# microsoft/vattention

Hardware: AMD Instinct MI355X
Metric: prefill+decode tokens/sec (attention + KV-memory hot path) (higher is better)
Workload: dtype f16

## Files before the change

vattention_amd/csrc/prefill64_common.h:

```cpp
#pragma once
#include "attn_common.h"

namespace vattn_k {

typedef float f32x2 __attribute__((ext_vector_type(2)));
constexpr float kDeferLog2 = 6.0f;

__device__ __forceinline__ void dma_piece(unsigned lds_addr, u32x4 rsrc, unsigned voff) {
    asm volatile("s_mov_b32 m0, %0\n\ts_nop 0\n\tbuffer_load_dwordx4 %2, %1, 0 offen lds" : : "s"(lds_addr), "s"(rsrc), "v"(voff) : "memory", "m0");
}
__device__ __forceinline__ void dma_piece_first(unsigned lds_addr, u32x4 rsrc, unsigned voff) {
    asm volatile("s_nop 4\n\ts_mov_b32 m0, %0\n\ts_nop 0\n\tbuffer_load_dwordx4 %2, %1, 0 offen lds" : : "s"(lds_addr), "s"(rsrc), "v"(voff) : "memory", "m0");
}
template <int OFF> __device__ __forceinline__ void dma_piece_at(unsigned lds_base, u32x4 rsrc, unsigned voff) {
    asm volatile("s_add_u32 m0, %0, %3\n\ts_nop 0\n\tbuffer_load_dwordx4 %2, %1, 0 offen lds" : : "s"(lds_base), "s"(rsrc), "v"(voff), "i"(OFF) : "memory", "m0", "scc");
}
template <int OFF, int ROWS> __device__ __forceinline__ void dma_piece_so(unsigned lds_base, u32x4 rsrc, unsigned voff, unsigned row_bytes) {
    unsigned so;
    asm volatile("s_add_u32 m0, %1, %6\n\ts_mul_i32 %0, %4, %5\n\tbuffer_load_dwordx4 %3, %2, %0 offen lds"
                 : "=&s"(so) : "s"(lds_base), "s"(rsrc), "v"(voff), "s"(row_bytes), "n"(ROWS), "i"(OFF) : "memory", "m0", "scc");
}
template <int ROWS> __device__ __forceinline__ unsigned piece_off(unsigned base, unsigned row_bytes) {
    unsigned r;
    asm("v_mad_u32_u24 %0, %1, %3, %2" : "=v"(r) : "s"(row_bytes), "v"(base), "n"(ROWS));
    return r;
}
__device__ __forceinline__ void k_rsrc_advance(u32x4& r, int& rows_left, unsigned tile_bytes, unsigned row_bytes) {
    asm volatile("s_add_u32 s92, s92, %3\n\ts_addc_u32 s93, s93, 0\n\ts_sub_i32 %1, %1, 64\n\ts_min_i32 s94, %1, 64\n\ts_max_i32 s94, s94, 0\n\ts_mul_i32 s94, s94, %4"
                 : "={s[92:95]}"(r), "+s"(rows_left) : "0"(r), "s"(tile_bytes), "s"(row_bytes) : "scc");
}
__device__ __forceinline__ void v_rsrc_advance(u32x4& r, int& rows_left, unsigned tile_bytes, unsigned row_bytes) {
    asm volatile("s_add_u32 s96, s96, %3\n\ts_addc_u32 s97, s97, 0\n\ts_sub_i32 %1, %1, 64\n\ts_min_i32 s98, %1, 64\n\ts_max_i32 s98, s98, 0\n\ts_mul_i32 s98, s98, %4"
                 : "={s[96:99]}"(r), "+s"(rows_left) : "0"(r), "s"(tile_bytes), "s"(row_bytes) : "scc");
}
__device__ __forceinline__ u32x4 tile_rsrc(const void* base, unsigned bytes) {
    const unsigned long long a = (unsigned long long)base;
    u32x4 r;
    r[0] = __builtin_amdgcn_readfirstlane((unsigned)a);
    r[1] = __builtin_amdgcn_readfirstlane((unsigned)(a >> 32)) & 0xffffu;
    r[2] = __builtin_amdgcn_readfirstlane(bytes);
    r[3] = 0x00020000u;
    return r;
}

template <typename T> struct Mfma;
#define VATTN_MFMA_STRUCT(TYPE, MNEM)                                                                                                    \
    template <> struct Mfma<TYPE> {                                                                                                \
        using V8 = typename Tr<TYPE>::v8;                                                                                          \
                                                                   \
        static __device__ __forceinline__ void qk_first(f32x16& d, V8 a, V8 b) {                                                   \
            asm volatile(MNEM " %0, %1, %2, 0" : "=&v"(d) : "v"(a), "a"(b));                                                       \
        }                                                                                                                          \
        static __device__ __forceinline__ void qk_acc(f32x16& d, V8 a, V8 b) {                                                     \
            asm volatile(MNEM " %0, %1, %2, %0" : "+v"(d) : "v"(a), "a"(b));                                                       \
        }                                                                                                                          \
                                                           \
        static __device__ __forceinline__ void qk_first_a(f32x16& d, V8 a, V8 b) {                                                 \
            asm volatile(MNEM " %0, %1, %2, 0" : "=&v"(d) : "a"(a), "a"(b));                                                       \
        }                                                                                                                          \
        static __device__ __forceinline__ void qk_acc_a(f32x16& d, V8 a, V8 b) {                                                   \
            asm volatile(MNEM " %0, %1, %2, %0" : "+v"(d) : "a"(a), "a"(b));                                                       \
        }                                                                                                                          \
                                                                                                 \
        static __device__ __forceinline__ void pv(f32x16& o, V8 a, V8 b) {                                                         \
            asm volatile(MNEM " %0, %1, %2, %0" : "+a"(o) : "v"(a), "v"(b));                                                       \
        }                                                                                                                          \
    };
VATTN_MFMA_STRUCT(_Float16, "v_mfma_f32_32x32x16_f16")
VATTN_MFMA_STRUCT(__bf16, "v_mfma_f32_32x32x16_bf16")
#undef VATTN_MFMA_STRUCT
__device__ __forceinline__ float add1(float a, float b) {
    float r;
    asm("v_add_f32 %0, %1, %2" : "=v"(r) : "v"(a), "v"(b));
    return r;
}
#define SCHED_FENCE() __builtin_amdgcn_sched_barrier(0)

constexpr int kKPiece = 1088;
constexpr int kKSlot = 16 * 1088;
constexpr int kVBase = 36864;

template <typename V8> __device__ __forceinline__ V8 kfrag(const char* ksm, int f, unsigned kfrag_lane) {
    const int kk = f >> 1, kb = f & 1;
    return *(const V8*)(ksm + kb * 8 * kKPiece + kk * 128 + kfrag_lane);
}
template <typename V8> __device__ __forceinline__ V8 vfrag(const char* vsm, int f, unsigned vfrag_lane) {
    const int ks = f >> 2, db = f & 3;
    const char* a1 = vsm + db * PfSmem<128>::kVSubBytes + (16 * ks) * 64 + vfrag_lane;
    const s16x4 lo = __builtin_amdgcn_ds_read_tr16_b64_v4i16(LDS_PTR(s16x4, a1));
    const s16x4 hi = __builtin_amdgcn_ds_read_tr16_b64_v4i16(LDS_PTR(s16x4, a1 + 8 * 64));
    return join_tr<V8>(lo, hi);
}
__device__ __forceinline__ float row_max(const f32x16 (&s)[2][2], int qc) {
    float m0 = fmaxf(s[0][qc][0], s[1][qc][0]);
#pragma unroll
    for (int r = 1; r < 16; r++) m0 = fmaxf(fmaxf(m0, s[0][qc][r]), s[1][qc][r]);
    return fmaxf(m0, swap_halves(m0));
}
template <int DB> __device__ __forceinline__ void raise_max(f32x16 (&o)[DB][2], float (&l_acc)[2][2], float (&nmsub)[2], int qc, float delta) {
    const float alpha = fast_exp2(-delta);
    nmsub[qc] -= delta;
#pragma unroll
    for (int i = 0; i < DB; i++)
#pragma unroll
        for (int r = 0; r < 16; r++) o[i][qc][r] *= alpha;
#pragma unroll
    for (int a4 = 0; a4 < 2; a4++) l_acc[qc][a4] *= alpha;
}
template <typename T> __device__ __forceinline__ typename Tr<T>::v8 pack_p(const f32x16 (&pt)[2][2], int ks, int qc) {
    typename Tr<T>::v8 r;
#pragma unroll
    for (int j = 0; j < 8; j++) r[j] = Tr<T>::cvt(pt[ks >> 1][qc][8 * (ks & 1) + j]);
    return r;
}
__device__ __forceinline__ unsigned bound(int rows, unsigned rs) {
    int r;
    asm("s_min_i32 %0, %1, 64\n\ts_max_i32 %0, %0, 0" : "=s"(r) : "s"(rows) : "scc");
    return (unsigned)r * rs;
}

template <int NA> __device__ __forceinline__ void softmax_stages(int G, f32x16 (&cur)[2][2], float (&l_acc)[2][2], const float (&nmsub)[2], unsigned escale_s) {
    auto GE = [](int e) { return e < NA ? 1 + (e * 30) / NA : 33 + ((e - NA) * 17) / (32 - NA); };
#define P64_X0(cur, e) cur[(e) >> 4][((e) >> 2) & 1][8 * (((e) >> 3) & 1) + 2 * ((e) & 3)]
#define P64_X1(cur, e) cur[(e) >> 4][((e) >> 2) & 1][8 * (((e) >> 3) & 1) + 2 * ((e) & 3) + 1]
#pragma unroll
    for (int e = 0; e < 32; e++) {
        const int qc = (e >> 2) & 1;
        if (GE(e) - 1 == G)
            asm("v_fma_f32 %0, %0, %2, %3\n\tv_fma_f32 %1, %1, %2, %3" : "+v"(P64_X0(cur, e)), "+v"(P64_X1(cur, e)) : "s"(escale_s), "v"(nmsub[qc]));
        if (GE(e) == G) asm("v_exp_f32 %0, %0\n\tv_exp_f32 %1, %1" : "+v"(P64_X0(cur, e)), "+v"(P64_X1(cur, e)));
        if (GE(e) + 1 == G)
            asm("v_add_f32 %0, %0, %2\n\tv_add_f32 %1, %1, %3" : "+v"(l_acc[qc][0]), "+v"(l_acc[qc][1]) : "v"(P64_X0(cur, e)), "v"(P64_X1(cur, e)));
    }
#undef P64_X0
#undef P64_X1
}

template <typename T, int KK> __device__ __forceinline__ void first_scores(const char* ksm, f32x16 (&sc)[2][2], const typename Tr<T>::v8 (&qf)[2][KK], unsigned kfrag_lane) {
    using V8 = typename Tr<T>::v8;
    using M = Mfma<T>;
#pragma unroll
    for (int f = 0; f < 2 * KK; f++) {
        const V8 a = kfrag<V8>(ksm, f, kfrag_lane);
#pragma unroll
        for (int qc = 0; qc < 2; qc++) {
            if (f < 2) M::qk_first(sc[f & 1][qc], a, qf[qc][f >> 1]);
            else M::qk_acc(sc[f & 1][qc], a, qf[qc][f >> 1]);
        }
    }
    asm volatile("s_nop 15\n\ts_nop 3" ::: "memory");
    SCHED_FENCE();
}

struct StepMax {
    float mx0, mx1, g0, g1, grow;
};
template <typename T, int NA, int RING, int MS, int BJ, int D0, int DS, typename Hook>
__device__ __forceinline__ StepMax tile_step(const int par, const char* smem, f32x16 (&cur)[2][2], f32x16 (&nxt)[2][2], typename Tr<T>::v8& kf0,
                                             typename Tr<T>::v8& kf1, typename Tr<T>::v8& kf2, const typename Tr<T>::v8 (&qf)[2][8], f32x16 (&o)[4][2],
                                             float (&l_acc)[2][2], const float (&nmsub)[2], u32x4& rk, u32x4& rv, int& k_rows_left, int& v_rows_left,
                                             unsigned& vs_cur, unsigned& vs_dma, unsigned k_lds_wave, unsigned v_lds_wave, unsigned koff, unsigned voff,
                                             unsigned k_rs_bytes, unsigned v_rs_bytes, unsigned k_tile_b, unsigned v_tile_b, unsigned kfrag_lane,
                                             unsigned vfrag_lane, unsigned escale_s, Hook hook) {
    using V8 = typename Tr<T>::v8;
    using M = Mfma<T>;
    using S = PfSmem<128>;
    constexpr int KK = 8;
    static_assert(D0 >= BJ && D0 + 7 * DS < 32, "DMA pieces behind the barrier, inside phase B");
    static_assert(NA >= 16 && NA < 32, "key slice 0 of P is packed in phase-A groups 13 / 15: its eight pairs must be exponentiated by group 12");
    static_assert(MS >= 4 && MS + 19 < 32, "row-max chain >= 4 MFMAs behind the last S^T MFMA, its reduction inside phase B");
    auto dma_gap = [](int k) { return D0 + DS * k; };
    const int s_cur = par;
    const char* ksm = smem + (s_cur ^ 1) * kKSlot;
    const char* ksm_next = smem + s_cur * kKSlot;
    const char* vsm = smem + kVBase + vs_cur;
    const unsigned lk0 = k_lds_wave + (unsigned)((s_cur ^ 1) * kKSlot);
    unsigned lv0 = 0;
    V8 pf[2][2];
    V8 kf[RING];
    V8 vf[RING];
    SCHED_FENCE();
#pragma unroll
    for (int i = 0; i < 32; i++) {
        const int f = i >> 1, qc = i & 1;
        if (f < RING - 1) {
            const V8 a = f == 0 ? kf0 : (f == 1 ? kf1 : kf2);
            if (i < 4) M::qk_first_a(nxt[f & 1][qc], a, qf[qc][f >> 1]);
            else M::qk_acc_a(nxt[f & 1][qc], a, qf[qc][f >> 1]);
        } else if (i < 4) M::qk_first(nxt[f & 1][qc], kf[f % RING], qf[qc][f >> 1]);
        else M::qk_acc(nxt[f & 1][qc], kf[f % RING], qf[qc][f >> 1]);
        if ((i & 1) == 0 && f + RING - 1 < 2 * KK) kf[(f + RING - 1) % RING] = kfrag<V8>(ksm, f + RING - 1, kfrag_lane);
        softmax_stages<NA>(i, cur, l_acc, nmsub, escale_s);
        if (i == 13) pf[0][0] = pack_p<T>(cur, 0, 0);
        if (i == 15) pf[0][1] = pack_p<T>(cur, 0, 1);
        if (i == 17) lv0 = v_lds_wave + vs_dma;
        if (i == 19) asm volatile("s_mov_b32 %1, %0\n\ts_add_u32 %0, %0, %2\n\ts_cmp_eq_u32 %0, %3\n\ts_cselect_b32 %0, 0, %0"
                                  : "+s"(vs_cur), "=&s"(vs_dma) : "i"(S::kTileBytes), "i"(3 * S::kTileBytes) : "scc");
        if (i == 21) k_rsrc_advance(rk, k_rows_left, k_tile_b, k_rs_bytes);
        if (i == 23) v_rsrc_advance(rv, v_rows_left, v_tile_b, v_rs_bytes);
        hook(i);
        if (i == 26) vf[0] = vfrag<V8>(vsm, 0, vfrag_lane);
        if (i == 28) vf[1] = vfrag<V8>(vsm, 1, vfrag_lane);
        if (i == 30 && RING > 3) vf[2] = vfrag<V8>(vsm, 2, vfrag_lane);
        SCHED_FENCE();
    }
    float mx0 = -INFINITY, mx1 = -INFINITY, g0 = -INFINITY, g1 = -INFINITY, grow = -INFINITY;
    SCHED_FENCE();
#pragma unroll
    for (int j = 0; j < 32; j++) {
        const int f = j >> 1, ks = j >> 3, qc = j & 1;
        if (j == BJ) {
            asm volatile("s_waitcnt vmcnt(0)" ::: "memory");
            __builtin_amdgcn_s_barrier();
        }
        M::pv(o[f & 3][qc], vf[f % RING], pf[ks & 1][qc]);
        if ((j & 1) == 0 && f + RING - 1 < 16) vf[(f + RING - 1) % RING] = vfrag<V8>(vsm, f + RING - 1, vfrag_lane);
        softmax_stages<NA>(32 + j, cur, l_acc, nmsub, escale_s);
        if (ks < 3 && (j & 7) == 4) pf[(ks + 1) & 1][0] = pack_p<T>(cur, ks + 1, 0);
        if (ks < 3 && (j & 7) == 6) pf[(ks + 1) & 1][1] = pack_p<T>(cur, ks + 1, 1);
        if (j >= MS && j < MS + 16) {
            const int r = j - MS;
            if (r == 0) {
                asm("v_max_f32_e32 %0, %1, %2" : "=v"(mx0) : "v"(nxt[0][0][0]), "v"(nxt[1][0][0]));
                asm("v_max_f32_e32 %0, %1, %2" : "=v"(mx1) : "v"(nxt[0][1][0]), "v"(nxt[1][1][0]));
            } else {
                asm("v_max3_f32 %0, %0, %1, %2" : "+v"(mx0) : "v"(nxt[0][0][r]), "v"(nxt[1][0][r]));
                asm("v_max3_f32 %0, %0, %1, %2" : "+v"(mx1) : "v"(nxt[0][1][r]), "v"(nxt[1][1][r]));
            }
        }
        if (j == MS + 16) mx0 = max_halves(mx0);
        if (j == MS + 17) mx1 = max_halves(mx1);
        if (j == MS + 18) {
            asm("v_fma_f32 %0, %2, %4, %5\n\tv_fma_f32 %1, %3, %4, %6" : "=&v"(g0), "=&v"(g1) : "v"(mx0), "v"(mx1), "s"(escale_s), "v"(nmsub[0]), "v"(nmsub[1]));
        }
        if (j == MS + 19) asm("v_max_f32 %0, %1, %2" : "=v"(grow) : "v"(g0), "v"(g1));
        if (j == dma_gap(0)) dma_piece_at<0>(lk0, rk, koff);
        if (j == dma_gap(1)) dma_piece_so<kKPiece, 4>(lk0, rk, koff, k_rs_bytes);
        if (j == dma_gap(2)) dma_piece_so<2 * kKPiece, 8>(lk0, rk, koff, k_rs_bytes);
        if (j == dma_gap(3)) dma_piece_so<3 * kKPiece, 12>(lk0, rk, koff, k_rs_bytes);
        if (j == dma_gap(4)) dma_piece_at<0>(lv0, rv, voff);
        if (j == dma_gap(5)) dma_piece_so<1024, 16>(lv0, rv, voff, v_rs_bytes);
        if (j == dma_gap(6)) dma_piece_so<2048, 32>(lv0, rv, voff, v_rs_bytes);
        if (j == dma_gap(7)) dma_piece_so<3072, 48>(lv0, rv, voff, v_rs_bytes);
        if (j == 27) kf0 = kfrag<V8>(ksm_next, 0, kfrag_lane);
        if (j == 28) kf1 = kfrag<V8>(ksm_next, 1, kfrag_lane);
        if (j == 29 && RING > 3) kf2 = kfrag<V8>(ksm_next, 2, kfrag_lane);
        SCHED_FENCE();
    }
    return {mx0, mx1, g0, g1, grow};
}

}
```

vattention_amd/csrc/prefill64_kernel.inc:

```
template <typename T>
__global__ __launch_bounds__(256, 1) void P64_KERNEL_NAME(vattn_attn_params p, int order, int nqb, int nsplit) {
    constexpr bool WIN = P64_WIN;
    constexpr int NA = 24, RING = 4, MS = 8, BJ = 8, D0 = 9, DS = 3;
    using X = Tr<T>;
    using V8 = typename X::v8;
    constexpr int HD = 128;
    using S = PfSmem<HD>;
    constexpr int BM = 256;
    constexpr int KK = HD / 16;
    constexpr int DB = HD / 32;
    extern __shared__ __attribute__((aligned(16))) char smem[];

    const int tid = threadIdx.x;
    const int lane = tid & 63;
    const int wave = __builtin_amdgcn_readfirstlane(tid >> 6);
    const int l31 = lane & 31;
    const int g = lane >> 5;

    int b, h, qb, split;
    const bool listed = p.pf_items != nullptr;
    int it_tb = 0, it_te = 0, it_row = -1;
    if (listed) {
        const vattn_prefill_item it = p.pf_items[blockIdx.x];
        b = __builtin_amdgcn_readfirstlane(it.b);
        h = __builtin_amdgcn_readfirstlane(it.h);
        qb = __builtin_amdgcn_readfirstlane(it.qb);
        it_tb = __builtin_amdgcn_readfirstlane(it.tile_begin);
        it_te = __builtin_amdgcn_readfirstlane(it.tile_end);
        it_row = __builtin_amdgcn_readfirstlane(it.nshares > 1 ? it.part_row : -1);
        split = 0;
    } else if (!wg_to_work(p, order, nqb, nsplit, b, h, qb, split)) return;
    const bool partial = listed ? it_row >= 0 : nsplit > 1;
    const int hk = h / (p.h / p.h_k);
    const int slot = __builtin_amdgcn_readfirstlane(p.cache_batch_idx ? p.cache_batch_idx[b] : b);
    int Lk = __builtin_amdgcn_readfirstlane((p.cache_seqlens ? p.cache_seqlens[b] : p.seqlen_k) + p.seqlen_knew);
    Lk = Lk > p.seqlen_k ? p.seqlen_k : Lk;
    const int Sq = p.q_lens ? __builtin_amdgcn_readfirstlane(p.q_lens[b]) : p.seqlen_q;
    const int64_t q_first = p.q_start ? (int64_t)__builtin_amdgcn_readfirstlane(p.q_start[b]) : 0;
    const bool causal = p.is_causal != 0;
    const int off = Lk - Sq;
    const int q_wg0 = qb * BM;
    if (q_wg0 >= Sq) return;
    const int qw0 = q_wg0 + wave * 64;

    int n_end = Lk;
    if (causal) n_end = min(Lk, q_wg0 + BM + off);
    if (n_end < 0) n_end = 0;
    const int nt_all = (n_end + PF_BN - 1) / PF_BN;
    const int left = WIN ? p.window_left_plus1 - 1 : 0;
    const int t_first = WIN ? min(nt_all, max(0, q_wg0 + off - left) >> 6) : 0;
    int tb = t_first, nt = nt_all;
    if (listed) {
        tb = min(nt_all, it_tb);
        nt = min(nt_all, it_te);
    } else if (nsplit > 1) {
        const int per = (nt_all - t_first + nsplit - 1) / nsplit;
        tb = min(nt_all, t_first + split * per);
        nt = min(nt_all, tb + per);
    }
    const T* kbase = uniform_ptr((const T*)p.k_cache + (int64_t)slot * p.k_batch_stride + (int64_t)hk * p.k_head_stride);
    const T* vbase = uniform_ptr((const T*)p.v_cache + (int64_t)slot * p.v_batch_stride + (int64_t)hk * p.v_head_stride);
    const unsigned k_rs_bytes = (unsigned)p.k_row_stride * 2u, v_rs_bytes = (unsigned)p.v_row_stride * 2u;

    unsigned koff[4], voff[4];
#pragma unroll
    for (int j = 0; j < 4; j++) {
        const int row = 4 * (4 * wave + j) + (lane & 3);
        koff[j] = (unsigned)row * k_rs_bytes + (unsigned)((lane >> 2) << 4);
        const int key = 16 * j + (lane >> 2);
        voff[j] = (unsigned)key * v_rs_bytes + (unsigned)((4 * wave + (lane & 3)) << 4);
    }
    const unsigned k_lds_wave = (unsigned)(wave * 4 * kKPiece);
    const unsigned v_lds_wave = (unsigned)(kVBase + wave * 4096);
    auto kslot = [&](int t) { return (t - tb) & 1; };
    auto k_rsrc = [&](int t) -> u32x4 {
        int rem = Lk - t * PF_BN;
        rem = rem < 0 ? 0 : (rem > PF_BN ? PF_BN : rem);
        return tile_rsrc(kbase + (int64_t)t * PF_BN * p.k_row_stride, (unsigned)rem * k_rs_bytes);
    };
    auto v_rsrc = [&](int t) -> u32x4 {
        int rem = Lk - t * PF_BN;
        rem = rem < 0 ? 0 : (rem > PF_BN ? PF_BN : rem);
        return tile_rsrc(vbase + (int64_t)t * PF_BN * p.v_row_stride, (unsigned)rem * v_rs_bytes);
    };
    auto dma_k_all = [&](int t) {
        const u32x4 r = k_rsrc(t);
        const unsigned l0 = k_lds_wave + (unsigned)(kslot(t) * kKSlot);
        dma_piece_first(l0, r, koff[0]);
        dma_piece(l0 + kKPiece, r, koff[1]);
        dma_piece(l0 + 2 * kKPiece, r, koff[2]);
        dma_piece(l0 + 3 * kKPiece, r, koff[3]);
    };
    auto dma_v_all = [&](int t) {
        const u32x4 r = v_rsrc(t);
        const unsigned l0 = v_lds_wave + (unsigned)(((t - tb) % 3) * S::kTileBytes);
        dma_piece_first(l0, r, voff[0]);
        dma_piece(l0 + 1024, r, voff[1]);
        dma_piece(l0 + 2048, r, voff[2]);
        dma_piece(l0 + 3072, r, voff[3]);
    };

    if (nt * PF_BN > Lk) {
        const uint4 z = make_uint4(0, 0, 0, 0);
#pragma unroll
        for (int i = 0; i < (3 * S::kTileBytes) / (256 * 16); i++) *(uint4*)(smem + kVBase + (i * 256 + tid) * 16) = z;
        __syncthreads();
    }
    dma_k_all(tb);
    dma_v_all(tb);
    dma_k_all(tb + 1);

    const float escale = p.softmax_scale * kLog2e;
    V8 qf[2][KK];
#pragma unroll
    for (int qc = 0; qc < 2; qc++) {
        const int my_q = qw0 + 32 * qc + l31;
        const T* qptr = (const T*)p.q + (p.q_start ? 0 : (int64_t)b * p.q_batch_stride) + (q_first + my_q) * p.q_row_stride + (int64_t)h * p.q_head_stride;
        V8 raw[KK];
#pragma unroll
        for (int kk = 0; kk < KK; kk++) {
            uint4 v = make_uint4(0, 0, 0, 0);
            if (my_q < Sq) {
                v = *(const uint4*)(qptr + 16 * kk + 8 * g);
            }
            raw[kk] = as_v8<V8>(v);
        }
        if (p.rotary_cos_sin && my_q < Sq && off + my_q >= 0) {
#pragma unroll
            for (int kk = 0; kk < KK / 2; kk++) {
                V8 c, s;
                rope_load<T>(p, (int64_t)(off + my_q), 16 * kk + 8 * g, c, s);
                rope8<T>(raw[kk], raw[kk + KK / 2], c, s);
            }
        }
#pragma unroll
        for (int kk = 0; kk < KK; kk++) {
            V8 sc8;
#pragma unroll
            for (int j = 0; j < 8; j++) sc8[j] = raw[kk][j];
            qf[qc][kk] = sc8;
            asm volatile("" : "+a"(qf[qc][kk]));
        }
    }

    f32x16 o[DB][2];
#pragma unroll
    for (int i = 0; i < DB; i++)
#pragma unroll
        for (int qc = 0; qc < 2; qc++) o[i][qc] = (f32x16){0.f, 0.f, 0.f, 0.f, 0.f, 0.f, 0.f, 0.f, 0.f, 0.f, 0.f, 0.f, 0.f, 0.f, 0.f, 0.f};
    float nmsub[2];
    float l_acc[2][2];
#pragma unroll
    for (int qc = 0; qc < 2; qc++) {
        nmsub[qc] = 0.f;
#pragma unroll
        for (int a4 = 0; a4 < 2; a4++) l_acc[qc][a4] = 0.f;
    }

    const unsigned kfrag_lane = (unsigned)((l31 >> 2) * kKPiece + (l31 & 3) * 16 + g * 64);
    const int i16 = lane & 15, dh = (lane >> 4) & 1;
    const unsigned vfrag_lane = (unsigned)((4 * g + (i16 >> 2)) * 64 + (16 * dh + 4 * (i16 & 3)) * 2);
    auto mask_tile = [&](int tt, f32x16 (&s)[2][2]) {
        const int n0 = tt * PF_BN;
#pragma unroll
        for (int qc = 0; qc < 2; qc++) {
            const int my_q = qw0 + 32 * qc + l31;
            const int lim = causal ? min(Lk - 1, my_q + off) : Lk - 1;
            const int lo = my_q + off - left;
#pragma unroll
            for (int kb = 0; kb < 2; kb++)
#pragma unroll
                for (int r = 0; r < 16; r++) {
                    const int key = n0 + 32 * kb + 8 * (r >> 2) + 4 * g + (r & 3);
                    if (WIN ? (unsigned)(key - lo) > (unsigned)left : key > lim) s[kb][qc][r] = -INFINITY;
                }
        }
    };
    const int t_mask = min(Lk >> 6, causal ? ((qw0 + off - 63) >> 6) + 1 : 0x7fffffff);
    const int t_lmask = WIN ? (qw0 + 63 + off - left) >> 6 : -1;
    auto needs_mask = [&](int tt) -> bool { return tt >= t_mask || (WIN && tt <= t_lmask); };
    auto first_vis = [&](int qc) -> int { return max(0, qw0 + 32 * qc + l31 + off - left) >> 6; };

    asm volatile("s_waitcnt vmcnt(8)" ::: "memory");
    __builtin_amdgcn_s_barrier();

    f32x16 sc[2][2];
    f32x16 sd[2][2];
    {
        first_scores<T>(smem + kslot(tb) * kKSlot, sc, qf, kfrag_lane);
        if (needs_mask(tb)) mask_tile(tb, sc);
#pragma unroll
        for (int qc = 0; qc < 2; qc++) {
            const float mx = row_max(sc, qc);
            nmsub[qc] = (mx == -INFINITY) ? 0.f : -mx * escale;
        }
    }

    const unsigned escale_s = __builtin_amdgcn_readfirstlane(__builtin_bit_cast(unsigned, escale));

    const unsigned k_tile_b = (unsigned)PF_BN * k_rs_bytes, v_tile_b = (unsigned)PF_BN * v_rs_bytes;
    int k_rows_left = Lk - (tb + 2) * PF_BN, v_rows_left = Lk - (tb + 1) * PF_BN;
    const unsigned long long kp0 = (unsigned long long)kbase + (unsigned long long)(tb + 2) * k_tile_b;
    const unsigned long long vp0 = (unsigned long long)vbase + (unsigned long long)(tb + 1) * v_tile_b;
    u32x4 rk = {(unsigned)kp0, (unsigned)(kp0 >> 32) & 0xffffu, bound(k_rows_left, k_rs_bytes), 0x00020000u};
    u32x4 rv = {(unsigned)vp0, (unsigned)(vp0 >> 32) & 0xffffu, bound(v_rows_left, v_rs_bytes), 0x00020000u};
    unsigned vs_cur = 0, vs_dma = 2 * S::kTileBytes;
    auto step = [&](int t, const int par, f32x16 (&cur)[2][2], f32x16 (&nxt)[2][2], V8& kf0, V8& kf1, V8& kf2) {
        auto [mx0, mx1, g0, g1, grow] = tile_step<T, NA, RING, MS, BJ, D0, DS>(par, smem, cur, nxt, kf0, kf1, kf2, qf, o, l_acc, nmsub, rk, rv, k_rows_left,
                                                                               v_rows_left, vs_cur, vs_dma, k_lds_wave, v_lds_wave, koff[0], voff[0], k_rs_bytes,
                                                                               v_rs_bytes, k_tile_b, v_tile_b, kfrag_lane, vfrag_lane, escale_s, [](int) {});
        if (needs_mask(t + 1)) {
            mask_tile(t + 1, nxt);
            mx0 = row_max(nxt, 0);
            mx1 = row_max(nxt, 1);
            if constexpr (WIN) {
                if (first_vis(0) == t + 1) nmsub[0] = (mx0 == -INFINITY) ? 0.f : -mx0 * escale;
                if (first_vis(1) == t + 1) nmsub[1] = (mx1 == -INFINITY) ? 0.f : -mx1 * escale;
            }
            g0 = __builtin_fmaf(mx0, escale, nmsub[0]);
            g1 = __builtin_fmaf(mx1, escale, nmsub[1]);
            grow = fmaxf(g0, g1);
        }
        if (__builtin_amdgcn_ballot_w64(grow > kDeferLog2) != 0) {
            asm volatile("s_nop 15\n\ts_nop 7" ::: "memory");
            SCHED_FENCE();
            raise_max(o, l_acc, nmsub, 0, fmaxf(g0, 0.f));
            raise_max(o, l_acc, nmsub, 1, fmaxf(g1, 0.f));
            SCHED_FENCE();
            asm volatile("s_nop 3" ::: "memory");
        }
    };
    asm volatile("s_waitcnt vmcnt(0)" ::: "memory");
    __builtin_amdgcn_s_barrier();
    dma_k_all(tb + 2);
    dma_v_all(tb + 1);
    const char* ksm1 = smem + kslot(tb + 1) * kKSlot;
    V8 kfa = kfrag<V8>(ksm1, 0, kfrag_lane), kfb = kfrag<V8>(ksm1, 1, kfrag_lane), kfc = kfrag<V8>(ksm1, 2, kfrag_lane);
    for (int t = tb; t < nt; t += 2) {
        step(t, 0, sc, sd, kfa, kfb, kfc);
        if (t + 1 < nt) step(t + 1, 1, sd, sc, kfa, kfb, kfc);
    }
    asm volatile("s_waitcnt vmcnt(0)\n\ts_nop 15\n\ts_nop 7" ::: "memory");
    SCHED_FENCE();

#pragma unroll
    for (int qc = 0; qc < 2; qc++) {
        const int my_q = qw0 + 32 * qc + l31;
        const float l_loc = l_acc[qc][0] + l_acc[qc][1];
        const float l_tot = l_loc + swap_halves(l_loc);
        const float inv = (l_tot == 0.f || l_tot != l_tot) ? 1.f : 1.f / l_tot;
        const float m_log2 = -nmsub[qc];
        auto part_row = [&](int q) -> int64_t {
            return listed ? (int64_t)it_row + (q - q_wg0) : (((int64_t)split * p.b + b) * p.seqlen_q + q) * p.h + h;
        };
        float* lpart = (float*)p.workspace + (listed ? (int64_t)p.pf_part_rows : (int64_t)nsplit * p.b * p.seqlen_q * p.h) * HD;
        if (my_q < Sq && partial) {
            const int64_t row = part_row(my_q);
            float* opart = (float*)p.workspace + row * HD;
#pragma unroll
            for (int db = 0; db < DB; db++)
#pragma unroll
                for (int tq = 0; tq < 4; tq++) {
                    f32x4 w;
#pragma unroll
                    for (int e = 0; e < 4; e++) w[e] = o[db][qc][4 * tq + e] * inv;
                    *(f32x4*)(opart + 32 * db + 8 * tq + 4 * g) = w;
                }
            if (g == 0) {
                const float lv = (l_tot == 0.f || l_tot != l_tot) ? -INFINITY : (m_log2 + __log2f(l_tot));
                lpart[row] = lv;
            }
        } else if (my_q < Sq) {
            T* optr = (T*)p.out + (p.q_start ? 0 : (int64_t)b * p.o_batch_stride) + (q_first + my_q) * p.o_row_stride + (int64_t)h * p.o_head_stride;
            if (((p.o_row_stride | p.o_head_stride | p.o_batch_stride) & 7) == 0) {
#pragma unroll
                for (int db = 0; db < DB; db++)
#pragma unroll
                    for (int pr = 0; pr < 2; pr++) {
                        typename X::v4 we, wo;
#pragma unroll
                        for (int e = 0; e < 4; e++) {
                            we[e] = X::cvt(o[db][qc][4 * (2 * pr) + e] * inv);
                            wo[e] = X::cvt(o[db][qc][4 * (2 * pr + 1) + e] * inv);
                        }
                        uint2 ue, uo;
                        __builtin_memcpy(&ue, &we, 8);
                        __builtin_memcpy(&uo, &wo, 8);
                        const auto r0 = __builtin_amdgcn_permlane32_swap(ue.x, uo.x, false, false);
                        const auto r1 = __builtin_amdgcn_permlane32_swap(ue.y, uo.y, false, false);
                        *(uint4*)(optr + 32 * db + 8 * (2 * pr + g)) = make_uint4(r0[0], r1[0], r0[1], r1[1]);
                    }
            } else {
#pragma unroll
                for (int db = 0; db < DB; db++)
#pragma unroll
                    for (int tq = 0; tq < 4; tq++) {
                        typename X::v4 w;
#pragma unroll
                        for (int e = 0; e < 4; e++) w[e] = X::cvt(o[db][qc][4 * tq + e] * inv);
                        *(typename X::v4*)(optr + 32 * db + 8 * tq + 4 * g) = w;
                    }
            }
            if (p.softmax_lse && g == 0) {
                const float lse = (l_tot == 0.f) ? INFINITY : (m_log2 + __log2f(l_tot)) * 0.6931471805599453f;
                p.softmax_lse[((int64_t)b * p.h + h) * p.seqlen_q + my_q] = lse;
            }
        }
    }
}
```

Measured before the change: 125,300.

## Skip fully masked causal tiles per wave while keeping cooperative DMA going

Each wave now computes how many K/V tiles it can actually see under the causal mask and runs the compute steps only up to that point. For the remaining tiles it still takes part in the cooperative DMA and barriers through a new carry_step helper, so the other waves in the block keep their loads and synchronisation. This removes wasted MFMA and softmax work on tiles that would be fully masked for early query rows. The output accumulators are also pinned to AGPRs at initialisation. The cost is extra control flow, and the skipped waves still pay for barrier waits.

```diff
diff --git a/vattention_amd/csrc/prefill64_common.h b/vattention_amd/csrc/prefill64_common.h
--- a/vattention_amd/csrc/prefill64_common.h
+++ b/vattention_amd/csrc/prefill64_common.h
@@ -250,4 +250,28 @@
     return {mx0, mx1, g0, g1, grow};
 }
 
-}
+__device__ __forceinline__ void carry_step(const int par, u32x4& rk, u32x4& rv, int& k_rows_left, int& v_rows_left, unsigned& vs_cur, unsigned& vs_dma,
+                                           unsigned k_lds_wave, unsigned v_lds_wave, unsigned koff, unsigned voff, unsigned k_rs_bytes, unsigned v_rs_bytes,
+                                           unsigned k_tile_b, unsigned v_tile_b) {
+    using S = PfSmem<128>;
+    const unsigned lk0 = k_lds_wave + (unsigned)((par ^ 1) * kKSlot);
+    SCHED_FENCE();
+    const unsigned lv0 = v_lds_wave + vs_dma;
+    asm volatile("s_mov_b32 %1, %0\n\ts_add_u32 %0, %0, %2\n\ts_cmp_eq_u32 %0, %3\n\ts_cselect_b32 %0, 0, %0"
+                 : "+s"(vs_cur), "=&s"(vs_dma) : "i"(S::kTileBytes), "i"(3 * S::kTileBytes) : "scc");
+    k_rsrc_advance(rk, k_rows_left, k_tile_b, k_rs_bytes);
+    v_rsrc_advance(rv, v_rows_left, v_tile_b, v_rs_bytes);
+    asm volatile("s_waitcnt vmcnt(0)" ::: "memory");
+    __builtin_amdgcn_s_barrier();
+    dma_piece_at<0>(lk0, rk, koff);
+    dma_piece_so<kKPiece, 4>(lk0, rk, koff, k_rs_bytes);
+    dma_piece_so<2 * kKPiece, 8>(lk0, rk, koff, k_rs_bytes);
+    dma_piece_so<3 * kKPiece, 12>(lk0, rk, koff, k_rs_bytes);
+    dma_piece_at<0>(lv0, rv, voff);
+    dma_piece_so<1024, 16>(lv0, rv, voff, v_rs_bytes);
+    dma_piece_so<2048, 32>(lv0, rv, voff, v_rs_bytes);
+    dma_piece_so<3072, 48>(lv0, rv, voff, v_rs_bytes);
+    SCHED_FENCE();
+}
+
+}
diff --git a/vattention_amd/csrc/prefill64_kernel.inc b/vattention_amd/csrc/prefill64_kernel.inc
--- a/vattention_amd/csrc/prefill64_kernel.inc
+++ b/vattention_amd/csrc/prefill64_kernel.inc
@@ -147,7 +147,10 @@
 #pragma unroll
     for (int i = 0; i < DB; i++)
 #pragma unroll
-        for (int qc = 0; qc < 2; qc++) o[i][qc] = (f32x16){0.f, 0.f, 0.f, 0.f, 0.f, 0.f, 0.f, 0.f, 0.f, 0.f, 0.f, 0.f, 0.f, 0.f, 0.f, 0.f};
+        for (int qc = 0; qc < 2; qc++) {
+            o[i][qc] = (f32x16){0.f, 0.f, 0.f, 0.f, 0.f, 0.f, 0.f, 0.f, 0.f, 0.f, 0.f, 0.f, 0.f, 0.f, 0.f, 0.f};
+            asm volatile("" : "+a"(o[i][qc]));
+        }
     float nmsub[2];
     float l_acc[2][2];
 #pragma unroll
@@ -178,6 +181,8 @@
     };
     const int t_mask = min(Lk >> 6, causal ? ((qw0 + off - 63) >> 6) + 1 : 0x7fffffff);
     const int t_lmask = WIN ? (qw0 + 63 + off - left) >> 6 : -1;
+    const int last_vis = causal ? min(Lk - 1, qw0 + 63 + off) : Lk - 1;
+    const int nt_wave = qw0 >= Sq ? 0 : min(nt, (last_vis >> 6) + 1);
     auto needs_mask = [&](int tt) -> bool { return tt >= t_mask || (WIN && tt <= t_lmask); };
     auto first_vis = [&](int qc) -> int { return max(0, qw0 + 32 * qc + l31 + off - left) >> 6; };
 
@@ -236,11 +241,18 @@
     dma_v_all(tb + 1);
     const char* ksm1 = smem + kslot(tb + 1) * kKSlot;
     V8 kfa = kfrag<V8>(ksm1, 0, kfrag_lane), kfb = kfrag<V8>(ksm1, 1, kfrag_lane), kfc = kfrag<V8>(ksm1, 2, kfrag_lane);
-    for (int t = tb; t < nt; t += 2) {
+    int t = tb;
+    while (t < nt_wave) {
         step(t, 0, sc, sd, kfa, kfb, kfc);
-        if (t + 1 < nt) step(t + 1, 1, sd, sc, kfa, kfb, kfc);
-    }
-    asm volatile("s_waitcnt vmcnt(0)\n\ts_nop 15\n\ts_nop 7" ::: "memory");
+        if (++t >= nt_wave) break;
+        step(t, 1, sd, sc, kfa, kfb, kfc);
+        t++;
+    }
+    asm volatile("s_nop 15\n\ts_nop 7" ::: "memory");
+    SCHED_FENCE();
+    for (; t < nt; t++)
+        carry_step((t - tb) & 1, rk, rv, k_rows_left, v_rows_left, vs_cur, vs_dma, k_lds_wave, v_lds_wave, koff[0], voff[0], k_rs_bytes, v_rs_bytes, k_tile_b, v_tile_b);
+    asm volatile("s_waitcnt vmcnt(0)" ::: "memory");
     SCHED_FENCE();
 
 #pragma unroll
```

After: 125,300, median of 2. Within noise of the previous version (+0.0%).
